# kalj/dealii-cuda

Hardware: AMD Instinct MI355X
Metric: DoFs/s on 1305x Laplace vmult (bmop), p=4 3D uniform (higher is better)
Workload: dtype f64; 1 GPU; bmop: DEGREE_FE=4, DIMENSION=3, MATRIX_FREE_UNIFORM_MESH, hyper_cube(-1,1), 54^3 cells, 10218313 DoFs, 1 z-slab(s); cells_per_dir=54, n_dofs=10218313, n_cells=157464, parallelism=slab1, dof_numbering=caller's (lexicographic), finite=True, clock_ramp_steps=2000

## Files before the change

dealii-cuda_amd/csrc/mfgpu_internal.h:

```cpp
#ifndef MFGPU_INTERNAL_H
#define MFGPU_INTERNAL_H

#include <cstdint>
#include <string>
#include <vector>

#include "../../include/mfgpu.h"

namespace mfgpu {

void set_error(const std::string &msg);

inline int ipow(int a, int e) {
  int r = 1;
  for (int i = 0; i < e; ++i) r *= a;
  return r;
}

constexpr int p_cells_per_wave(int n) { return 64 / n; }
constexpr int p_ji(int n) { return n == 3 ? 2 : n == 4 ? 5 : n == 5 ? 9 : n == 6 ? 14 : 23; }
constexpr int p_hs(int n) { return n == 3 ? 3 : n == 4 ? 6 : n == 5 ? 9 : n == 6 ? 14 : 18; }
constexpr int p_kgu(int n) { return p_ji(n) + p_hs(n); }
constexpr int p_cell_stride(int n) {
  int s = n * n * n;
  while ((s & 31) != (n & 31)) ++s;
  return s;
}

constexpr int q_plane_stride(int n) { return n >= 6 ? 65 : n == 5 ? 33 : n == 4 ? 17 : 33; }
constexpr int q_cell_stride(int n) { return n * q_plane_stride(n); }
constexpr int p_priv_max(int n) { return n >= 5 ? 384 : n == 4 ? 256 : 192; }
constexpr int kHnOpRounds = 2;
constexpr int p_hn_rows(int n) { return p_priv_max(n) / 64 + 3 * kHnOpRounds * 3 + 2; }

template <typename T>
constexpr size_t q_region_doubles(int n) {
  const size_t t = ((size_t)(p_cells_per_wave(n) + 1) * q_cell_stride(n) * sizeof(T) + 7) / 8;
  const size_t u = (size_t)p_kgu(n) * 64 + p_priv_max(n);
  return t > u ? t : u;
}
template <typename T>
constexpr size_t q_lds_bytes(int n, bool hn) {
  return (q_region_doubles<T>(n) + (hn ? (size_t)n * n : 0)) * 8;
}

constexpr uint8_t kFlagConstrained = 1;
constexpr uint8_t kFlagAdd = 2;

struct Plan {
  int dim = 0, degree = 0, n = 0, nd = 0;
  uint32_t n_dofs = 0, n_cells = 0;
  std::vector<uint32_t> cell_order;
  std::vector<uint32_t> batch_cell_off;
  std::vector<uint32_t> batch_dof_off;
  std::vector<uint32_t> color_batch_off;
  std::vector<uint32_t> bdofs;
  std::vector<uint8_t> bflags;
  std::vector<uint16_t> lmap;
  std::vector<uint32_t> orphans;
  std::vector<uint32_t> batch_nint;
  std::vector<uint32_t> halo_off;
  std::vector<uint32_t> sdofs;
  std::vector<uint32_t> s_off;
  std::vector<uint32_t> s_idx;
  std::vector<uint32_t> chunks;
  std::vector<uint32_t> gstarts;
  uint32_t max_batch_dofs = 0, max_batch_cells = 0;
  uint32_t n_plane_batches = 0;
  uint32_t n_plain_plane_batches = 0;
  std::vector<uint32_t> pr_dofs, pr_idx, pr_hn, pr_hn_slot;
  std::vector<uint32_t> sh_dofs, sh_idx, sh_batch;
  bool sh_use = false;
  std::vector<uint32_t> sh_p2rec, sh_p2tab;
  bool sh_p2_use = false;
  uint64_t n_first = 0, n_add = 0;
};

struct PlanLimits {
  uint32_t max_cells = 0, max_dofs = 0;
  uint32_t interior_max = 0, shared_max = 0, halo_stride = 0;
  bool segregate_masked = false;
  bool masked_planes = false;
  uint32_t private_max = 0;
};

int build_plan(const mfgpu_desc &d, Plan &plan, uint32_t max_chunks = 3, const PlanLimits *limits = nullptr);

struct HnLine {
  uint16_t node[8];
};
void hn_cell_lines(unsigned mask, int n, std::vector<HnLine> (&lines)[3], std::vector<uint16_t> &nodes);

enum class PlaneKernel : uint8_t { none, planes3, planes4 };
enum class BatchKernel : uint8_t { none, batches, x, g, g2 };
int choose_kernel_and_plan(const mfgpu_desc &d, PlaneKernel &pk, BatchKernel &bk, Plan &plan);

constexpr bool planes4_wide(int n) { return n >= 6; }
constexpr bool kernel_exists(PlaneKernel k, int n, int number_type, bool hn, bool sh, bool mass) {
  switch (k) {
    case PlaneKernel::planes3: return n >= 3 && n <= 5 && !(sh && hn);
    case PlaneKernel::planes4:
      return planes4_wide(n) ? n <= 7 && !hn && !sh && !mass
                             : n >= 3 && !sh && !(mass && n == 5 && number_type == MFGPU_F64);
    default: return false;
  }
}
constexpr bool kernel_exists(BatchKernel k, int n, int , bool , bool sh, bool ) {
  return k != BatchKernel::none && n >= 2 && n <= 7 && !sh;
}
constexpr int kFusedWidths[] = {3, 2};
constexpr bool fused_kernel_exists(BatchKernel k, int n, int number_type, bool hn, bool , int nv) {
  return k == BatchKernel::g && n >= 2 && n <= 7 && (nv == 2 || nv == 3) &&
         !(hn && number_type == MFGPU_F64 && n >= (nv == 3 ? 6 : 7));
}
std::vector<uint32_t> multi_groups(uint32_t n_vectors, const std::vector<uint32_t> &widths);
int build_plane_records(Plan &plan, const uint32_t *constraint_mask);
constexpr int kShBatchWords = 4;
constexpr double kShareMaxFraction = 0.5;
void share_plane_records(Plan &plan);
constexpr int kP2Header = 16, kP2MaxK = 12, kP2SlotBits = 12;
void share_pass2_records(Plan &plan);

std::vector<uint16_t> x_lane_permutation(int n);
std::vector<uint16_t> x_pencil_runs(const std::vector<uint16_t> &lmap, int n);
struct Pass2Group {
  std::vector<uint32_t> dofs, offsets = std::vector<uint32_t>(1, 0u), slots;
};
int pass2_groups(const Plan &plan, const std::vector<uint32_t> &seg_end, const uint32_t *priority, uint32_t n_priority,
                 bool shared, std::vector<Pass2Group> &groups);

int derive_tables(int n, const double *shape_values, const double *shape_gradients,
                  std::vector<double> &S, std::vector<double> &Dt);

int handle_number_type(const mfgpu_handle *h);
int handle_set_priority_dofs(mfgpu_handle *h, const uint32_t *ids, uint32_t n);
int handle_vmult_phase(mfgpu_handle *h, int phase, void *dst, const void *src, void *stream, int add);
int handle_n_batches(const mfgpu_handle *h);
bool handle_ranged_ok(const mfgpu_handle *h);
int handle_batches_touching(const mfgpu_handle *h, const uint32_t *ids, uint32_t n, std::vector<uint8_t> &flags);
int handle_cells_range(mfgpu_handle *h, uint32_t b0, uint32_t b1, void *dst, const void *src, void *stream, int add);
int handle_cells_two_ranges(mfgpu_handle *h, uint32_t b0, uint32_t b1, uint32_t c0, uint32_t c1, void *dst,
                            const void *src, void *stream, int add);
int handle_pass2_group(mfgpu_handle *h, int group, void *dst, const void *src, void *stream, int add);

void transfer_sizes(const mfgpu_transfer *t, uint32_t *n_coarse_dofs, uint32_t *n_fine_dofs, int *number_type);
void vcycle_active(const mfgpu_vcycle *v, int *active_type, uint32_t *n_active);

}

struct mfgpu_plan {
  mfgpu::Plan plan;
};

#endif
```

dealii-cuda_amd/csrc/mfgpu_kernels_p.hip:

```cpp
#include <hip/hip_runtime.h>

#include "mfgpu_cell.h"
#include "mfgpu_kernels.h"
#include "mfgpu_planes.h"

namespace mfgpu {

#define MFGPU_PIN_VMEM() __builtin_amdgcn_sched_barrier(0x380)

template <int n, typename T, bool ADD, bool HN, bool SH = false, bool MASS = false>
__global__ void __launch_bounds__(64) __attribute__((amdgpu_waves_per_eu(1, 1)))
apply_planes3(const ApplyArgs<T> A, const TablesEO<T, n> tab) {
  constexpr int n2 = n * n;
  constexpr int CW = p_cells_per_wave(n);
  constexpr int NT = CW * n;
  constexpr int KGU = p_kgu(n);
  constexpr int JI = p_ji(n);
  constexpr int HS = KGU - JI;
  constexpr int SA = p_cell_stride(n);
  constexpr int NIW = (n2 + 1) / 2;
  extern __shared__ __attribute__((aligned(16))) unsigned char smem_raw[];
  constexpr int PRIV = HN ? p_priv_max(n) : 0;
  double *ua = reinterpret_cast<double *>(smem_raw);
  T *Aw = reinterpret_cast<T *>(ua + KGU * 64 + PRIV + (HN ? n2 : 0));
  T *Bw = Aw + (CW + 1) * SA;
  double *Wl = ua + KGU * 64 + PRIV;

  const int lane = threadIdx.x;
  if (HN) {
    if (lane < n2) Wl[lane] = (double)A.hn_weights[lane];
  }
  const int lc = lane / n, k = lane - lc * n;
  const bool lane_on = lane < NT;
  const int tk = lane_on ? lane : NT - 1;

  uint32_t b, bstride, bend;
  {
    const uint32_t nbt = A.batch_end - A.batch0 - A.hole_len, G = gridDim.x;
    if (G >= 8 && nbt >= G) {
      const uint32_t xcd = blockIdx.x & 7u, slot = blockIdx.x >> 3;
      const uint32_t q = G >> 3, rem = G & 7u;
      const uint32_t wlo = xcd * q + (xcd < rem ? xcd : rem);
      const uint32_t w = q + (xcd < rem ? 1u : 0u);
      b = A.batch0 + (uint32_t)((uint64_t)nbt * wlo / G) + slot;
      bend = A.batch0 + (uint32_t)((uint64_t)nbt * (wlo + w) / G);
      bstride = w;
    } else {
      b = A.batch0 + blockIdx.x;
      bend = A.batch_end - A.hole_len;
      bstride = G;
    }
  }
  if (b >= bend) return;
  const uint32_t hole0 = A.hole0, hole_len = A.hole_len;
  auto next_of = [&](uint32_t x) {
    const uint32_t l = (x >= hole0 ? x - hole_len : x) + bstride;
    return l < bend ? (l >= hole0 ? l + hole_len : l) : x;
  };
  if (b >= hole0) b += hole_len;
  static_assert(kernel_exists(PlaneKernel::planes3, n, number_type_of<T>, HN, SH, MASS), "no such instantiation");
  struct Meta {
    uint32_t base, drec, irec;
  };
  auto meta_request = [&](uint32_t bb) -> uint32_t {
    return A.shtab[(size_t)bb * kShBatchWords + (lane & (kShBatchWords - 1))];
  };
  auto meta_of = [&](uint32_t v) -> Meta {
    return Meta{(uint32_t)__builtin_amdgcn_readlane((int)v, 0), (uint32_t)__builtin_amdgcn_readlane((int)v, 1),
                (uint32_t)__builtin_amdgcn_readlane((int)v, 2)};
  };

  auto load_dofs = [&](uint32_t rec, uint32_t (&g)[KGU]) {
    const uint32_t *p = A.bdofsp + (size_t)rec * (KGU * 64) + lane;
#pragma unroll
    for (int j = 0; j < KGU; ++j) g[j] = SH ? p[j * 64] : nt_load(p + j * 64);
  };
  auto src_at = [&](uint32_t base, uint32_t g) -> T {
    const T *const sp = SH ? A.src + base : A.src;
    return *reinterpret_cast<const T *>(reinterpret_cast<const char *>(sp) + (uint32_t)(g * (uint32_t)sizeof(T)));
  };
  auto dst_at = [&](uint32_t base, uint32_t g) -> T * {
    T *const dp = SH ? A.dst + base : A.dst;
    return reinterpret_cast<T *>(reinterpret_cast<char *>(dp) + (uint32_t)(g * (uint32_t)sizeof(T)));
  };
  auto load_ix = [&](uint32_t rec, uint32_t (&ix)[NIW]) {
    const uint32_t *p = A.idxp + (size_t)rec * (NIW * NT) + tk;
#pragma unroll
    for (int w = 0; w < NIW; ++w) ix[w] = SH ? p[w * NT] : nt_load(p + w * NT);
  };
  auto stage_src = [&](const uint32_t (&g)[KGU], const T (&sv)[KGU]) {
#pragma unroll
    for (int j = 0; j < KGU; ++j) {
      double v = (double)sv[j];
      if (j >= JI) {
        const unsigned long long keep = (unsigned long long)(long long)~((int)g[j] >> 31);
        v = __longlong_as_double((long long)((unsigned long long)__double_as_longlong(v) & keep));
      }
      ua[lane + j * 64] = v;
    }
  };
  auto ixb = [&](const uint32_t (&ix)[NIW], int i) -> uint32_t {
    return (i & 1) ? (ix[i >> 1] >> 16) : (ix[i >> 1] & 0xffffu);
  };
  auto scatter_slot = [&](int j, uint32_t bb, uint32_t base, uint32_t g, T r, T oldv) {
    if (j < JI) {
      *dst_at(base, g) = ADD ? oldv + r : r;
    } else {
      T *const hp = A.halo + (size_t)bb * (HS * 64) + lane;
      hp[(j - JI) * 64] = r;
    }
  };

  uint32_t b1 = next_of(b), b2 = next_of(b1);
  uint32_t Gp[KGU], Gc[KGU], Gn[KGU], Gnn[KGU];
  uint32_t IXc[NIW], IXn[NIW];
  constexpr int CR = PRIV / 64, HROWS = HN ? p_hn_rows(n) : 1;
  uint32_t Hc[HROWS], Hn[HROWS];
  auto load_hn = [&](uint32_t bb, uint32_t (&H)[HROWS]) {
    const uint32_t slot = A.hn_slot[bb];
    if (slot != 0xffffffffu) {
      const uint32_t *p = A.hnrec + (size_t)slot * (HROWS * 64) + lane;
#pragma unroll
      for (int w = 0; w < HROWS; ++w) H[w] = nt_load(p + w * 64);
    } else {
#pragma unroll
      for (int w = 0; w < HROWS; ++w) H[w] = 0u;
    }
  };
  T Cc[n2];
  T Mm[MASS ? n2 : 1];
  T SVn[KGU], R[KGU], old[KGU];
  Meta Mp{0u, 0u, 0u}, Mc = Mp, M1 = Mp, M2 = Mp;
  uint32_t Mv = 0u;
  if (SH) {
    Mc = meta_of(meta_request(b));
    M1 = meta_of(meta_request(b1));
    M2 = meta_of(meta_request(b2));
    Mp = Mc;
  }
  load_dofs(SH ? Mc.drec : b, Gc);
  load_dofs(SH ? M1.drec : b1, Gn);
  load_ix(SH ? Mc.irec : b, IXc);
  if (HN) load_hn(b, Hc);
  constexpr uint32_t kDummyIx = 8u * (uint32_t)(KGU * 64 - 1) * 0x10001u;
#pragma unroll
  for (int w = 0; w < NIW; ++w) IXc[w] = lane_on ? IXc[w] : kDummyIx;
  {
    const T *p = A.coefp + (size_t)b * (n2 * NT) + tk;
#pragma unroll
    for (int r = 0; r < n2; ++r) Cc[r] = nt_load(p + r * NT);
  }
  if (MASS) {
    const T *p = A.massp + (size_t)b * (n2 * NT) + tk;
#pragma unroll
    for (int r = 0; r < n2; ++r) Mm[r] = nt_load(p + r * NT);
  }
#pragma unroll
  for (int j = 0; j < KGU; ++j) {
    SVn[j] = src_at(Mc.base, Gc[j]);
    Gp[j] = Gc[j];
    R[j] = T(0);
    old[j] = T(0);
  }
  stage_src(Gc, SVn);
  WaveSync::sync();

  const int pxy = lc * SA + n2 * k;
  const int pyz = lc * SA + k;
  uint32_t bp = b;

  while (true) {
    const bool has_next = b1 != b;
    constexpr int kH2 = HN ? HROWS - 2 : 0, kH1 = HN ? HROWS - 1 : 0;
    const uint32_t hn_ncopy = HN ? (uint32_t)__builtin_amdgcn_readfirstlane(Hc[kH2] & 0xffffu) : 0u;
    auto hn_count = [&](int dir) -> uint32_t {
      const uint32_t w = dir == 0 ? Hc[kH2] >> 16 : dir == 1 ? Hc[kH1] & 0xffffu : Hc[kH1] >> 16;
      return (uint32_t)__builtin_amdgcn_readfirstlane(w);
    };
    auto hn_pass = [&](int dir, bool transposed, const double (&Wr)[n2]) {
      const uint32_t count = hn_count(dir);
#pragma unroll
      for (int r = 0; r < kHnOpRounds; ++r) {
        if ((uint32_t)(r * 64) >= count) break;
        const bool on = (uint32_t)(r * 64 + lane) < count;
        const uint32_t *ww = &Hc[CR + (dir * kHnOpRounds + r) * 3];
        double v[n], o[n];
        uint32_t pos[n];
#pragma unroll
        for (int t = 0; t < n; ++t) {
          pos[t] = on ? (ww[t >> 1] >> (16 * (t & 1))) & 0xffffu : (uint32_t)(KGU * 64 + PRIV - 1);
          v[t] = ua[pos[t]];
        }
#pragma unroll
        for (int i = 0; i < n; ++i) {
          double acc = 0.0;
#pragma unroll
          for (int k2 = 0; k2 < n; ++k2) acc = fma(transposed ? Wr[k2 * n + i] : Wr[i * n + k2], v[k2], acc);
          o[i] = acc;
        }
        if (on) {
#pragma unroll
          for (int i = 0; i < n; ++i) ua[pos[i]] = o[i];
        }
      }
    };
    if (HN && hn_ncopy) {
      double Wr[n2];
#pragma unroll
      for (int i = 0; i < n2; ++i) Wr[i] = Wl[i];
      double cv[CR > 0 ? CR : 1];
#pragma unroll
      for (int r = 0; r < CR; ++r) cv[r] = (uint32_t)(r * 64 + lane) < hn_ncopy ? ua[Hc[r] & 0xffffu] : 0.0;
#pragma unroll
      for (int r = 0; r < CR; ++r)
        if ((uint32_t)(r * 64 + lane) < hn_ncopy) ua[Hc[r] >> 16] = cv[r];
      WaveSync::sync();
      hn_pass(0, false, Wr);
      WaveSync::sync();
      hn_pass(1, false, Wr);
      WaveSync::sync();
      hn_pass(2, false, Wr);
      WaveSync::sync();
    }
    STAMP(0);
    RSTAMP(8);
    WGSTAMP(10);
    load_dofs(SH ? M2.drec : b2, Gnn);
    load_ix(SH ? M1.irec : b1, IXn);
    if (SH) Mv = meta_request(next_of(b2));
    if (HN) load_hn(b1, Hn);
    if (ADD) {
#pragma unroll
      for (int j = 0; j < JI; ++j) old[j] = *dst_at(Mp.base, Gp[j]);
    }
    STAMP(1);
    auto hookA = [&](int) {};
    auto hookB = [&](int s) {
      MFGPU_PIN_VMEM();
#pragma unroll
      for (int j = (KGU * s) / (5 * n); j < (KGU * (s + 1)) / (5 * n); ++j)
        scatter_slot(j, bp, Mp.base, Gp[j], R[j], old[j]);
#pragma unroll
      for (int j = (KGU * s) / (5 * n); j < (KGU * (s + 1)) / (5 * n); ++j)
        SVn[j] = src_at(M1.base, Gn[j]);
      MFGPU_PIN_VMEM();
    };
    const T *const cnext = A.coefp + (size_t)b1 * (n2 * NT) + tk;
    const T *const mnext = MASS ? A.massp + (size_t)b1 * (n2 * NT) + tk : nullptr;
    auto hookC = [&](int s) {
      MFGPU_PIN_VMEM();
#pragma unroll
      for (int r = (n2 * s) / (2 * n); r < (n2 * (s + 1)) / (2 * n); ++r)
        Cc[r] = nt_load(cnext + r * NT);
      if (MASS) {
#pragma unroll
        for (int r = (n2 * s) / (2 * n); r < (n2 * (s + 1)) / (2 * n); ++r)
          Mm[r] = nt_load(mnext + r * NT);
      }
      MFGPU_PIN_VMEM();
    };

    {
      T u[n2];
#pragma unroll
      for (int x = 0; x < n; ++x)
#pragma unroll
        for (int y = 0; y < n; ++y)
          u[x + n * y] = (T) * reinterpret_cast<const double *>(reinterpret_cast<const char *>(ua) + ixb(IXc, x + n * y));
#pragma unroll
      for (int x = 0; x < n; ++x) {
        T in[n], out[n];
        get_line<n, 1>(u, x, in);
        eo_apply<n, 0>(tab, in, out);
        set_line<n, 1>(u, x, out);
        hookA(x);
      }
#pragma unroll
      for (int y = 0; y < n; ++y) {
        T in[n], a[n], bb[n];
        get_line<n, 0>(u, y, in);
        eo_apply<n, 0>(tab, in, a);
        eo_apply<n, 2>(tab, a, bb);
#pragma unroll
        for (int x = 0; x < n; ++x) {
          Aw[pxy + x + n * y] = a[x];
          Bw[pxy + x + n * y] = bb[x];
        }
        hookA(n + y);
      }
    }
    WaveSync::sync();
    STAMP(2);
#pragma unroll
    for (int j = 0; j < KGU + PRIV / 64; ++j) ua[lane + j * 64] = 0.0;

    {
      T nx[n];
#pragma unroll
      for (int z = 0; z < n; ++z) nx[z] = Bw[pyz + n2 * z];
#pragma unroll
      for (int y = 0; y < n; ++y) {
        T in[n], g[n], o[n];
#pragma unroll
        for (int z = 0; z < n; ++z) in[z] = nx[z];
#pragma unroll
        for (int z = 0; z < n; ++z) nx[z] = y + 1 < n ? Bw[pyz + n * (y + 1) + n2 * z] : Aw[pyz + n2 * z];
        eo_apply<n, 0>(tab, in, g);
#pragma unroll
        for (int z = 0; z < n; ++z) g[z] *= Cc[y + n * z];
        eo_apply<n, 1>(tab, g, o);
#pragma unroll
        for (int z = 0; z < n; ++z) Bw[pyz + n * y + n2 * z] = o[z];
        hookB(y);
      }
      T v[n2], r[n2];
#pragma unroll
      for (int y = 0; y < n; ++y) {
        T in[n], o[n];
#pragma unroll
        for (int z = 0; z < n; ++z) in[z] = nx[z];
        if (y + 1 < n) {
#pragma unroll
          for (int z = 0; z < n; ++z) nx[z] = Aw[pyz + n * (y + 1) + n2 * z];
        }
        eo_apply<n, 0>(tab, in, o);
        set_line<n, 1>(v, y, o);
        hookB(n + y);
      }
#pragma unroll
      for (int y = 0; y < n; ++y) {
        T in[n], g[n], o[n];
        get_line<n, 1>(v, y, in);
        eo_apply<n, 2>(tab, in, g);
#pragma unroll
        for (int z = 0; z < n; ++z) g[z] *= Cc[y + n * z];
        eo_apply<n, 3>(tab, g, o);
        set_line<n, 1>(r, y, o);
        hookB(2 * n + y);
      }
#pragma unroll
      for (int z = 0; z < n; ++z) {
        T in[n], g[n], o[n];
        get_line<n, 0>(v, z, in);
        eo_apply<n, 2>(tab, in, g);
#pragma unroll
        for (int y = 0; y < n; ++y) g[y] *= Cc[y + n * z];
        eo_apply<n, 3>(tab, g, o);
#pragma unroll
        for (int y = 0; y < n; ++y) r[y + n * z] += MASS ? fma(Mm[y + n * z], in[y], o[y]) : o[y];
        hookB(3 * n + z);
      }
#pragma unroll
      for (int y = 0; y < n; ++y) {
        T in[n], o[n];
        get_line<n, 1>(r, y, in);
        eo_apply<n, 1>(tab, in, o);
#pragma unroll
        for (int z = 0; z < n; ++z) Aw[pyz + n * y + n2 * z] = o[z];
        hookB(4 * n + y);
      }
    }
    WaveSync::sync();
    STAMP(3);

    {
      T o[n2];
      T nr[n], nt[n];
#pragma unroll
      for (int x = 0; x < n; ++x) {
        nr[x] = Aw[pxy + x];
        nt[x] = Bw[pxy + x];
      }
#pragma unroll
      for (int y = 0; y < n; ++y) {
        T rp[n], tp[n], w[n], ol[n];
#pragma unroll
        for (int x = 0; x < n; ++x) {
          rp[x] = nr[x];
          tp[x] = nt[x];
        }
        if (y + 1 < n) {
#pragma unroll
          for (int x = 0; x < n; ++x) {
            nr[x] = Aw[pxy + x + n * (y + 1)];
            nt[x] = Bw[pxy + x + n * (y + 1)];
          }
        }
        eo_apply<n, 3>(tab, tp, w);
#pragma unroll
        for (int x = 0; x < n; ++x) w[x] += rp[x];
        eo_apply<n, 1>(tab, w, ol);
        set_line<n, 0>(o, y, ol);
        hookC(y);
      }
#pragma unroll
      for (int x = 0; x < n; ++x) {
        T in[n], out[n];
        get_line<n, 1>(o, x, in);
        eo_apply<n, 1>(tab, in, out);
#pragma unroll
        for (int y = 0; y < n; ++y)
          lds_add(reinterpret_cast<double *>(reinterpret_cast<char *>(ua) + ixb(IXc, x + n * y)), (double)out[y]);
        hookC(n + x);
      }
    }
    WaveSync::sync();
    STAMP(4);

    if (HN && hn_ncopy) {
      double Wr[n2];
#pragma unroll
      for (int i = 0; i < n2; ++i) Wr[i] = Wl[i];
      hn_pass(2, true, Wr);
      WaveSync::sync();
      hn_pass(1, true, Wr);
      WaveSync::sync();
      hn_pass(0, true, Wr);
      WaveSync::sync();
      double cv[CR > 0 ? CR : 1];
#pragma unroll
      for (int r = 0; r < CR; ++r) cv[r] = (uint32_t)(r * 64 + lane) < hn_ncopy ? ua[Hc[r] >> 16] : 0.0;
#pragma unroll
      for (int r = 0; r < CR; ++r)
        if ((uint32_t)(r * 64 + lane) < hn_ncopy) lds_add(ua + (Hc[r] & 0xffffu), cv[r]);
      WaveSync::sync();
    }
#pragma unroll
    for (int j = 0; j < KGU; ++j) R[j] = (T)ua[lane + j * 64];
    WaveSync::sync();
    STAMP(5);
    stage_src(Gn, SVn);
    STAMP(6);
    bp = b;
    if (SH) Mp = Mc;
#pragma unroll
    for (int j = 0; j < KGU; ++j) Gp[j] = Gc[j];
    STAMP(7);
    RSTAMP(9);
    if (!has_next) break;
    WaveSync::sync();
    b = b1;
    b1 = b2;
    b2 = next_of(b2);
    if (SH) {
      Mc = M1;
      M1 = M2;
      M2 = meta_of(Mv);
    }
#pragma unroll
    for (int j = 0; j < KGU; ++j) {
      Gc[j] = Gn[j];
      Gn[j] = Gnn[j];
    }
#pragma unroll
    for (int w = 0; w < NIW; ++w) IXc[w] = lane_on ? IXn[w] : kDummyIx;
    if (HN) {
#pragma unroll
      for (int w = 0; w < HROWS; ++w) Hc[w] = Hn[w];
    }
  }
  if (ADD) {
#pragma unroll
    for (int j = 0; j < JI; ++j) old[j] = *dst_at(Mp.base, Gp[j]);
  }
#pragma unroll
  for (int j = 0; j < KGU; ++j) scatter_slot(j, bp, Mp.base, Gp[j], R[j], old[j]);
}

template <int n, typename T>
static size_t p_lds_bytes(bool hn) {
  return ((size_t)p_kgu(n) * 64 + (hn ? (size_t)p_priv_max(n) + n * n : 0)) * sizeof(double) +
         (size_t)2 * (p_cells_per_wave(n) + 1) * p_cell_stride(n) * sizeof(T);
}

template <typename T>
hipError_t p_bind(int, int n, bool hn, bool, bool sh, bool mass, uint32_t, CellKernel<T> *k) {
  return dispatch_instantiation(n, [&](auto N, auto HN, auto SH, auto MASS) {
    constexpr int n_ = N;
    if constexpr (kernel_exists(PlaneKernel::planes3, n_, number_type_of<T>, HN, SH, MASS))
      return bind_cell_kernel<T, 64, apply_planes3<n_, T, false, HN, SH, MASS>, apply_planes3<n_, T, true, HN, SH, MASS>,
                              make_tables_eo<T, n_>>(p_lds_bytes<n_, T>(HN), k);
    else
      return hipErrorInvalidValue;
  }, hn, sh, mass);
}
template hipError_t p_bind<double>(int, int, bool, bool, bool, bool, uint32_t, CellKernel<double> *);
template hipError_t p_bind<float>(int, int, bool, bool, bool, bool, uint32_t, CellKernel<float> *);

template <typename T>
__global__ void relayout_coef_kernel(T *out, const T *in, const uint32_t *cell_batch, const uint32_t *cell_pos,
                                     size_t total, int n) {
  const size_t i = (size_t)blockIdx.x * blockDim.x + threadIdx.x;
  if (i >= total) return;
  const int n2 = n * n, nd = n2 * n, NT = (64 / n) * n;
  const size_t cell = i / nd;
  const int q = (int)(i - cell * nd);
  const int x = q % n, r = q / n;
  out[((size_t)cell_batch[cell] * n2 + r) * NT + cell_pos[cell] * n + x] = in[i];
}

template <typename T>
hipError_t relayout_coef_launch(T *out, const T *in, const uint32_t *cell_batch, const uint32_t *cell_pos,
                                size_t total, int n, hipStream_t st) {
  if (total == 0) return hipSuccess;
  hipLaunchKernelGGL(relayout_coef_kernel<T>, dim3((unsigned)((total + 255) / 256)), dim3(256), 0, st, out, in,
                     cell_batch, cell_pos, total, n);
  return hipGetLastError();
}
template hipError_t relayout_coef_launch<double>(double *, const double *, const uint32_t *, const uint32_t *, size_t,
                                                 int, hipStream_t);
template hipError_t relayout_coef_launch<float>(float *, const float *, const uint32_t *, const uint32_t *, size_t, int,
                                                hipStream_t);

}
```

Baseline: 80.33 billion DoFs/s.

## Use bank-conflict-free row layout for planes3 LDS transpose buffers at n=5 f64

Adds an alternative LDS layout for the planes3 kernel's two transpose arrays when n=5, f64 and no hanging nodes. Rows use a stride of 31 with x mirrored, and idle lanes mirror active lanes, so the xy and yz plane views avoid LDS bank conflicts. Compile-time checks verify injectivity, affine addressing and conflict freedom, and confirm that four workgroups still fit in a CU's LDS. The cost is a separate index array for idle lanes' lds_add targets and slightly different LDS sizing.

```diff
diff --git a/dealii-cuda_amd/csrc/mfgpu_internal.h b/dealii-cuda_amd/csrc/mfgpu_internal.h
--- a/dealii-cuda_amd/csrc/mfgpu_internal.h
+++ b/dealii-cuda_amd/csrc/mfgpu_internal.h
@@ -26,12 +26,111 @@
   while ((s & 31) != (n & 31)) ++s;
   return s;
 }
+constexpr int kTrRowStride = 31;
+constexpr bool p_tr_rows(int n, size_t elem_bytes, bool hn) { return n == 5 && elem_bytes == 8 && !hn; }
+constexpr int p_tr_index(bool rows, int n, int c, int x, int y, int z) {
+  return rows ? kTrRowStride * (n * c + z) + (n - 1 - x) + n * y : c * p_cell_stride(n) + x + n * y + n * n * z;
+}
+constexpr int p_tr_base_xy(bool rows, int n, int c, int k) { return p_tr_index(rows, n, c, rows ? n - 1 : 0, 0, k); }
+constexpr int p_tr_base_yz(bool rows, int n, int c, int k) { return p_tr_index(rows, n, c, k, 0, 0); }
+constexpr int p_tr_xy(bool rows, int n, int x, int y) { return p_tr_index(rows, n, 0, x, y, 0) - p_tr_base_xy(rows, n, 0, 0); }
+constexpr int p_tr_yz(bool rows, int n, int y, int z) { return p_tr_index(rows, n, 0, 0, y, z) - p_tr_base_yz(rows, n, 0, 0); }
+struct TrView {
+  int per_c, per_k, base0, imm0, per_a, per_b;
+};
+constexpr TrView p_tr_view_xy(bool rows, int n) {
+  return TrView{p_tr_base_xy(rows, n, 1, 0) - p_tr_base_xy(rows, n, 0, 0),
+                p_tr_base_xy(rows, n, 0, 1) - p_tr_base_xy(rows, n, 0, 0),
+                p_tr_base_xy(rows, n, 0, 0),
+                p_tr_xy(rows, n, 0, 0),
+                p_tr_xy(rows, n, 1, 0) - p_tr_xy(rows, n, 0, 0),
+                p_tr_xy(rows, n, 0, 1) - p_tr_xy(rows, n, 0, 0)};
+}
+constexpr TrView p_tr_view_yz(bool rows, int n) {
+  return TrView{p_tr_base_yz(rows, n, 1, 0) - p_tr_base_yz(rows, n, 0, 0),
+                p_tr_base_yz(rows, n, 0, 1) - p_tr_base_yz(rows, n, 0, 0),
+                p_tr_base_yz(rows, n, 0, 0),
+                p_tr_yz(rows, n, 0, 0),
+                p_tr_yz(rows, n, 1, 0) - p_tr_yz(rows, n, 0, 0),
+                p_tr_yz(rows, n, 0, 1) - p_tr_yz(rows, n, 0, 0)};
+}
+constexpr int p_tr_len(bool rows, int n) {
+  return rows ? kTrRowStride * (n * p_cells_per_wave(n) - 1) + n * n : (p_cells_per_wave(n) + 1) * p_cell_stride(n);
+}
+constexpr int p_tr_mirror(int n, int lane) {
+  return lane < n * p_cells_per_wave(n) ? lane : lane - (64 - n * p_cells_per_wave(n));
+}
+
+namespace tr_check {
+constexpr bool injective(bool rows, int n) {
+  const int cells = p_cells_per_wave(n), len = p_tr_len(rows, n);
+  bool seen[4096] = {};
+  for (int c = 0; c < cells; ++c)
+    for (int z = 0; z < n; ++z)
+      for (int y = 0; y < n; ++y)
+        for (int x = 0; x < n; ++x) {
+          const int i = p_tr_index(rows, n, c, x, y, z);
+          if (i < 0 || i >= len || seen[i]) return false;
+          seen[i] = true;
+        }
+  return true;
+}
+constexpr bool affine(bool rows, int n) {
+  const TrView xy = p_tr_view_xy(rows, n), yz = p_tr_view_yz(rows, n);
+  for (int c = 0; c <= p_cells_per_wave(n); ++c)
+    for (int k = 0; k < n; ++k)
+      for (int a = 0; a < n; ++a)
+        for (int b = 0; b < n; ++b) {
+          const int pxy = c * xy.per_c + xy.per_k * k + xy.base0, ixy = xy.imm0 + xy.per_a * a + xy.per_b * b;
+          const int pyz = c * yz.per_c + yz.per_k * k + yz.base0, iyz = yz.imm0 + yz.per_a * a + yz.per_b * b;
+          if (ixy < 0 || iyz < 0) return false;
+          if (pxy + ixy != p_tr_index(rows, n, c, a, b, k) || pyz + iyz != p_tr_index(rows, n, c, k, a, b)) return false;
+        }
+  return true;
+}
+constexpr bool group_free(int n, bool yz, int lo, int width, int banks) {
+  for (int a = 0; a < n; ++a)
+    for (int b = 0; b < n; ++b) {
+      int addr_of_bank[64] = {};
+      for (int i = 0; i < 64; ++i) addr_of_bank[i] = -1;
+      for (int lane = lo; lane < lo + width; ++lane) {
+        const int m = p_tr_mirror(n, lane), c = m / n, k = m - c * n;
+        const int addr = yz ? p_tr_base_yz(true, n, c, k) + p_tr_yz(true, n, a, b)
+                            : p_tr_base_xy(true, n, c, k) + p_tr_xy(true, n, a, b);
+        if (addr != p_tr_index(true, n, c, yz ? k : a, yz ? a : b, yz ? b : k)) return false;
+        int &slot = addr_of_bank[addr % banks];
+        if (slot >= 0 && slot != addr) return false;
+        slot = addr;
+      }
+    }
+  return true;
+}
+constexpr bool view_free(int n, bool yz) {
+  for (int g = 0; g < 2; ++g)
+    if (!group_free(n, yz, 32 * g, 32, 32)) return false;
+  for (int g = 0; g < 4; ++g)
+    if (!group_free(n, yz, 16 * g, 16, 16)) return false;
+  return true;
+}
+}
+static_assert(tr_check::injective(true, 5) && tr_check::injective(false, 5), "transpose layout: two elements on one address");
+static_assert(tr_check::affine(true, 5) && tr_check::affine(false, 5) && tr_check::affine(false, 4) &&
+                  tr_check::affine(false, 3),
+              "transpose layout: base + immediate is not the element's index");
+static_assert(tr_check::view_free(5, false), "row layout: bank conflict in the xy-plane view");
+static_assert(tr_check::view_free(5, true), "row layout: bank conflict in the yz-plane view");
 
 constexpr int q_plane_stride(int n) { return n >= 6 ? 65 : n == 5 ? 33 : n == 4 ? 17 : 33; }
 constexpr int q_cell_stride(int n) { return n * q_plane_stride(n); }
 constexpr int p_priv_max(int n) { return n >= 5 ? 384 : n == 4 ? 256 : 192; }
 constexpr int kHnOpRounds = 2;
 constexpr int p_hn_rows(int n) { return p_priv_max(n) / 64 + 3 * kHnOpRounds * 3 + 2; }
+constexpr size_t p_lds_bytes(int n, size_t elem_bytes, bool hn) {
+  return ((size_t)p_kgu(n) * 64 + (hn ? (size_t)p_priv_max(n) + n * n : 0)) * sizeof(double) +
+         (size_t)2 * p_tr_len(p_tr_rows(n, elem_bytes, hn), n) * elem_bytes;
+}
+static_assert(p_tr_len(true, 5) == 1854 && p_lds_bytes(5, 8, false) == 38880, "row layout: size");
+static_assert(p_lds_bytes(5, 8, false) <= 40960, "four plane workgroups no longer fit the LDS of a CU");
 
 template <typename T>
 constexpr size_t q_region_doubles(int n) {
diff --git a/dealii-cuda_amd/csrc/mfgpu_kernels_p.hip b/dealii-cuda_amd/csrc/mfgpu_kernels_p.hip
--- a/dealii-cuda_amd/csrc/mfgpu_kernels_p.hip
+++ b/dealii-cuda_amd/csrc/mfgpu_kernels_p.hip
@@ -8,7 +8,8 @@
 
 #define MFGPU_PIN_VMEM() __builtin_amdgcn_sched_barrier(0x380)
 
-template <int n, typename T, bool ADD, bool HN, bool SH = false, bool MASS = false>
+template <int n, typename T, bool ADD, bool HN, bool SH = false, bool MASS = false,
+          bool TR = p_tr_rows(n, sizeof(T), HN)>
 __global__ void __launch_bounds__(64) __attribute__((amdgpu_waves_per_eu(1, 1)))
 apply_planes3(const ApplyArgs<T> A, const TablesEO<T, n> tab) {
   constexpr int n2 = n * n;
@@ -17,22 +18,25 @@
   constexpr int KGU = p_kgu(n);
   constexpr int JI = p_ji(n);
   constexpr int HS = KGU - JI;
-  constexpr int SA = p_cell_stride(n);
   constexpr int NIW = (n2 + 1) / 2;
   extern __shared__ __attribute__((aligned(16))) unsigned char smem_raw[];
   constexpr int PRIV = HN ? p_priv_max(n) : 0;
   double *ua = reinterpret_cast<double *>(smem_raw);
+  static_assert(TR == p_tr_rows(n, sizeof(T), HN), "p_lds_bytes sizes the arrays for this layout");
   T *Aw = reinterpret_cast<T *>(ua + KGU * 64 + PRIV + (HN ? n2 : 0));
-  T *Bw = Aw + (CW + 1) * SA;
+  constexpr int TL = p_tr_len(TR, n);
+  T *Bw = Aw + TL;
   double *Wl = ua + KGU * 64 + PRIV;
 
   const int lane = threadIdx.x;
   if (HN) {
     if (lane < n2) Wl[lane] = (double)A.hn_weights[lane];
   }
-  const int lc = lane / n, k = lane - lc * n;
+  const int lm = TR ? (lane < NT ? lane : lane - (64 - NT)) : lane;
+  static_assert(!TR || 2 * NT >= 64, "an idle lane mirrors a lane with a task");
+  const int lc = lm / n, k = lm - lc * n;
   const bool lane_on = lane < NT;
-  const int tk = lane_on ? lane : NT - 1;
+  const int tk = TR ? lm : lane_on ? lane : NT - 1;
 
   uint32_t b, bstride, bend;
   {
@@ -114,6 +118,7 @@
   uint32_t b1 = next_of(b), b2 = next_of(b1);
   uint32_t Gp[KGU], Gc[KGU], Gn[KGU], Gnn[KGU];
   uint32_t IXc[NIW], IXn[NIW];
+  uint32_t IXa[TR ? NIW : 1];
   constexpr int CR = PRIV / 64, HROWS = HN ? p_hn_rows(n) : 1;
   uint32_t Hc[HROWS], Hn[HROWS];
   auto load_hn = [&](uint32_t bb, uint32_t (&H)[HROWS]) {
@@ -144,7 +149,12 @@
   if (HN) load_hn(b, Hc);
   constexpr uint32_t kDummyIx = 8u * (uint32_t)(KGU * 64 - 1) * 0x10001u;
 #pragma unroll
-  for (int w = 0; w < NIW; ++w) IXc[w] = lane_on ? IXc[w] : kDummyIx;
+  for (int w = 0; w < NIW; ++w) {
+    if constexpr (TR)
+      IXa[w] = lane_on ? IXc[w] : kDummyIx;
+    else
+      IXc[w] = lane_on ? IXc[w] : kDummyIx;
+  }
   {
     const T *p = A.coefp + (size_t)b * (n2 * NT) + tk;
 #pragma unroll
@@ -165,8 +175,11 @@
   stage_src(Gc, SVn);
   WaveSync::sync();
 
-  const int pxy = lc * SA + n2 * k;
-  const int pyz = lc * SA + k;
+  constexpr TrView VXY = p_tr_view_xy(TR, n), VYZ = p_tr_view_yz(TR, n);
+  const int pxy = lc * VXY.per_c + VXY.per_k * k + VXY.base0;
+  const int pyz = lc * VYZ.per_c + VYZ.per_k * k + VYZ.base0;
+#define P_XY(x, y) (pxy + VXY.imm0 + VXY.per_a * (x) + VXY.per_b * (y))
+#define P_YZ(y, z) (pyz + VYZ.imm0 + VYZ.per_a * (y) + VYZ.per_b * (z))
   uint32_t bp = b;
 
   while (true) {
@@ -283,8 +296,8 @@
         eo_apply<n, 2>(tab, a, bb);
 #pragma unroll
         for (int x = 0; x < n; ++x) {
-          Aw[pxy + x + n * y] = a[x];
-          Bw[pxy + x + n * y] = bb[x];
+          Aw[P_XY(x, y)] = a[x];
+          Bw[P_XY(x, y)] = bb[x];
         }
         hookA(n + y);
       }
@@ -297,20 +310,20 @@
     {
       T nx[n];
 #pragma unroll
-      for (int z = 0; z < n; ++z) nx[z] = Bw[pyz + n2 * z];
+      for (int z = 0; z < n; ++z) nx[z] = Bw[P_YZ(0, z)];
 #pragma unroll
       for (int y = 0; y < n; ++y) {
         T in[n], g[n], o[n];
 #pragma unroll
         for (int z = 0; z < n; ++z) in[z] = nx[z];
 #pragma unroll
-        for (int z = 0; z < n; ++z) nx[z] = y + 1 < n ? Bw[pyz + n * (y + 1) + n2 * z] : Aw[pyz + n2 * z];
+        for (int z = 0; z < n; ++z) nx[z] = y + 1 < n ? Bw[P_YZ(y + 1, z)] : Aw[P_YZ(0, z)];
         eo_apply<n, 0>(tab, in, g);
 #pragma unroll
         for (int z = 0; z < n; ++z) g[z] *= Cc[y + n * z];
         eo_apply<n, 1>(tab, g, o);
 #pragma unroll
-        for (int z = 0; z < n; ++z) Bw[pyz + n * y + n2 * z] = o[z];
+        for (int z = 0; z < n; ++z) Bw[P_YZ(y, z)] = o[z];
         hookB(y);
       }
       T v[n2], r[n2];
@@ -321,7 +334,7 @@
         for (int z = 0; z < n; ++z) in[z] = nx[z];
         if (y + 1 < n) {
 #pragma unroll
-          for (int z = 0; z < n; ++z) nx[z] = Aw[pyz + n * (y + 1) + n2 * z];
+          for (int z = 0; z < n; ++z) nx[z] = Aw[P_YZ(y + 1, z)];
         }
         eo_apply<n, 0>(tab, in, o);
         set_line<n, 1>(v, y, o);
@@ -356,7 +369,7 @@
         get_line<n, 1>(r, y, in);
         eo_apply<n, 1>(tab, in, o);
 #pragma unroll
-        for (int z = 0; z < n; ++z) Aw[pyz + n * y + n2 * z] = o[z];
+        for (int z = 0; z < n; ++z) Aw[P_YZ(y, z)] = o[z];
         hookB(4 * n + y);
       }
     }
@@ -368,8 +381,8 @@
       T nr[n], nt[n];
 #pragma unroll
       for (int x = 0; x < n; ++x) {
-        nr[x] = Aw[pxy + x];
-        nt[x] = Bw[pxy + x];
+        nr[x] = Aw[P_XY(x, 0)];
+        nt[x] = Bw[P_XY(x, 0)];
       }
 #pragma unroll
       for (int y = 0; y < n; ++y) {
@@ -382,8 +395,8 @@
         if (y + 1 < n) {
 #pragma unroll
           for (int x = 0; x < n; ++x) {
-            nr[x] = Aw[pxy + x + n * (y + 1)];
-            nt[x] = Bw[pxy + x + n * (y + 1)];
+            nr[x] = Aw[P_XY(x, y + 1)];
+            nt[x] = Bw[P_XY(x, y + 1)];
           }
         }
         eo_apply<n, 3>(tab, tp, w);
@@ -400,7 +413,10 @@
         eo_apply<n, 1>(tab, in, out);
 #pragma unroll
         for (int y = 0; y < n; ++y)
-          lds_add(reinterpret_cast<double *>(reinterpret_cast<char *>(ua) + ixb(IXc, x + n * y)), (double)out[y]);
+          if constexpr (TR)
+            lds_add(reinterpret_cast<double *>(reinterpret_cast<char *>(ua) + ixb(IXa, x + n * y)), (double)out[y]);
+          else
+            lds_add(reinterpret_cast<double *>(reinterpret_cast<char *>(ua) + ixb(IXc, x + n * y)), (double)out[y]);
         hookC(n + x);
       }
     }
@@ -453,7 +469,14 @@
       Gn[j] = Gnn[j];
     }
 #pragma unroll
-    for (int w = 0; w < NIW; ++w) IXc[w] = lane_on ? IXn[w] : kDummyIx;
+    for (int w = 0; w < NIW; ++w) {
+      if constexpr (TR) {
+        IXc[w] = IXn[w];
+        IXa[w] = lane_on ? IXn[w] : kDummyIx;
+      } else {
+        IXc[w] = lane_on ? IXn[w] : kDummyIx;
+      }
+    }
     if (HN) {
 #pragma unroll
       for (int w = 0; w < HROWS; ++w) Hc[w] = Hn[w];
@@ -466,12 +489,8 @@
 #pragma unroll
   for (int j = 0; j < KGU; ++j) scatter_slot(j, bp, Mp.base, Gp[j], R[j], old[j]);
 }
-
-template <int n, typename T>
-static size_t p_lds_bytes(bool hn) {
-  return ((size_t)p_kgu(n) * 64 + (hn ? (size_t)p_priv_max(n) + n * n : 0)) * sizeof(double) +
-         (size_t)2 * (p_cells_per_wave(n) + 1) * p_cell_stride(n) * sizeof(T);
-}
+#undef P_XY
+#undef P_YZ
 
 template <typename T>
 hipError_t p_bind(int, int n, bool hn, bool, bool sh, bool mass, uint32_t, CellKernel<T> *k) {
@@ -479,7 +498,7 @@
     constexpr int n_ = N;
     if constexpr (kernel_exists(PlaneKernel::planes3, n_, number_type_of<T>, HN, SH, MASS))
       return bind_cell_kernel<T, 64, apply_planes3<n_, T, false, HN, SH, MASS>, apply_planes3<n_, T, true, HN, SH, MASS>,
-                              make_tables_eo<T, n_>>(p_lds_bytes<n_, T>(HN), k);
+                              make_tables_eo<T, n_>>(p_lds_bytes(n_, sizeof(T), HN), k);
     else
       return hipErrorInvalidValue;
   }, hn, sh, mass);
```

Measured after the change: 80.55 billion DoFs/s (median of 6 runs). Within noise of the previous version (+0.3%).
